# visinf/da-sac

Hardware: AMD Instinct MI355X
Metric: train images/sec (769x769, 19-cls, RN101 DeepLabv2, K=3) (higher is better)
Workload: dtype f32

## Files before the change

### da-sac_amd/csrc/winograd.hip

```cpp
#include "conv_common.hpp"
#include "winograd_index.hpp"

namespace dasac {
namespace wino {

constexpr int kBlock = 256;

__device__ __forceinline__ float ld(__amdgpu_buffer_rsrc_t r, unsigned voff) {
  return __uint_as_float(__builtin_amdgcn_raw_buffer_load_b32(r, voff, 0, 0));
}
__device__ __forceinline__ void st(__amdgpu_buffer_rsrc_t r, unsigned voff, float v) {
  __builtin_amdgcn_raw_buffer_store_b32(__float_as_uint(v), r, voff, 0, 0);
}

__global__ __launch_bounds__(kBlock) void filter_transform(const float* __restrict__ Wt, const float* __restrict__ scale,
                                                            float* __restrict__ U, int Cout, int Cin, int Mpad, int Kpad, int mode,
                                                            unsigned w_bytes, unsigned u_bytes) {
  const int idx = blockIdx.x * kBlock + threadIdx.x;
  const int per_point = Kpad * Mpad;
  if (idx >= per_point) return;
  const __amdgpu_buffer_rsrc_t rw = make_rsrc(Wt, w_bytes), ru = make_rsrc(U, u_bytes);
  const int row4 = Mpad * 4;
  const int kq = idx / row4, rem = idx - kq * row4;
  const int m = rem >> 2, k = kq * 4 + (rem & 3);
// ... 136 lines not shown
    for (int s = c; s < splits; s += 64) sv += ld(rs, (unsigned)(s * M + co) * 4u);
    sv = wave_sum(sv);
    if (c == 0) st(make_rsrc(sum_dz, (unsigned)M * 4u), (unsigned)co * 4u, sv);
  }
  __shared__ float red[4][16][64];
  __shared__ float grad[64 * 9];
  float acc[16];
#pragma unroll
  for (int pt = 0; pt < 16; ++pt) acc[pt] = 0.f;
  const unsigned point = (unsigned)(M * C), slab = 16u * point;
  const unsigned e0 = (unsigned)(co * C + ci0 + c);
  for (int s = q; s < splits; s += 4)
#pragma unroll
    for (int pt = 0; pt < 16; ++pt) acc[pt] += ld(rp, ((unsigned)s * slab + (unsigned)pt * point + e0) * 4u);
#pragma unroll
  for (int pt = 0; pt < 16; ++pt) red[q][pt][c] = acc[pt];
  __syncthreads();
  if (q == 0) {
    float p[4][4];
#pragma unroll
    for (int pt = 0; pt < 16; ++pt) p[pt >> 2][pt & 3] = (red[0][pt][c] + red[1][pt][c]) + (red[2][pt][c] + red[3][pt][c]);
    float r[3][4];
#pragma unroll
    for (int b = 0; b < 4; ++b) {
      r[0][b] = p[0][b] + 0.5f * (p[1][b] + p[2][b]);
      r[1][b] = 0.5f * (p[1][b] - p[2][b]);
      r[2][b] = 0.5f * (p[1][b] + p[2][b]) + p[3][b];
    }
#pragma unroll
    for (int a = 0; a < 3; ++a) {
      grad[c * 9 + a * 3 + 0] = r[a][0] + 0.5f * (r[a][1] + r[a][2]);
      grad[c * 9 + a * 3 + 1] = 0.5f * (r[a][1] - r[a][2]);
      grad[c * 9 + a * 3 + 2] = 0.5f * (r[a][1] + r[a][2]) + r[a][3];
    }
  }
  __syncthreads();
  const float sc = scale ? ld(make_rsrc(scale, (unsigned)M * 4u), (unsigned)co * 4u) : 1.f;
  float part = 0.f;
  for (int e = tx; e < 64 * 9; e += kBlock) {
    const unsigned off = ((unsigned)(co * C + ci0) * 9u + (unsigned)e) * 4u;
    if (dot) part += grad[e] * ld(rw, off);
    st(rd, off, grad[e] * sc);
  }
  if (dot) {
    __shared__ float redd[4];
    part = wave_sum(part);
    if (c == 0) redd[q] = part;
    __syncthreads();
    if (tx == 0) st(make_rsrc(dot, (unsigned)((C / 64) * M) * 4u), (unsigned)(blockIdx.x * M + co) * 4u, (redd[0] + redd[1]) + (redd[2] + redd[3]));
  }
}

}
}

using namespace dasac;
using dasac::wino::Geom;

static int wino_geom(Geom& g, const char* who, int Nb, int C, int M, int H, int W, int dilation) {
  DASAC_REQUIRE(Nb > 0 && C > 0 && M > 0 && H > 0 && W > 0 && dilation > 0, "%s: bad geometry", who);
  DASAC_REQUIRE((int64_t)Nb * H * W < (1ll << 30), "%s: more than 2^30 pixels", who);
  g = wino::make_geom(Nb, H, W, dilation);
  const int64_t cmax = C > M ? C : M;
  DASAC_REQUIRE(16 * cmax * (int64_t)g.T * 4 <= wino::kMaxBytes && cmax * (int64_t)Nb * H * W * 4 <= wino::kMaxBytes,
                "%s: a tensor exceeds the 4 GiB buffer-descriptor window", who);
  return DASAC_OK;
// ... 68 lines not shown

extern "C" int dasac_winograd_grad_input(const float* dz, int Nb, int M, int H, int W, int dilation, float* dm, size_t dm_bytes,
                                         dasac_stream_t stream) {
  DASAC_REQUIRE(dz && dm, "winograd_grad_input: null pointer");
  Geom g;
  const int rc = wino_geom(g, "winograd_grad_input", Nb, M, M, H, W, dilation);
  if (rc) return rc;
  DASAC_REQUIRE(M <= 65535, "winograd_grad_input: more than 65535 channels");
  const size_t need = (size_t)16 * M * g.T * 4;
  if (dm_bytes < need) return fail(DASAC_EWORKSPACE, "winograd_grad_input: workspace too small (%zu < %zu)", dm_bytes, need);
  hipLaunchKernelGGL(wino::grad_transform, dim3((g.T + wino::kBlock - 1) / wino::kBlock, M), dim3(wino::kBlock), 0, as_stream(stream), dz,
                     dm, g, M, (unsigned)((int64_t)Nb * M * H * W * 4), (unsigned)need);
  DASAC_CHECK_LAUNCH("winograd grad_transform");
  return DASAC_OK;
}

extern "C" int dasac_winograd_wgrad_finish(const void* workspace, size_t ws_bytes, int M, int C, int T, const float* w,
                                           const float* scale, float* dw, float* dot, float* sum_dz, dasac_stream_t stream) {
  DASAC_REQUIRE(workspace && w && dw, "winograd_wgrad_finish: null pointer");
  DASAC_REQUIRE(M > 0 && M <= 65535 && C > 0 && C % 64 == 0, "winograd_wgrad_finish: needs 1..65535 output channels and a multiple of 64 input channels");
  const int splits = dasac_conv_wgrad_batched_splits(16, M, C, T);
  DASAC_REQUIRE(splits > 0, "winograd_wgrad_finish: the batched weight-gradient launch does not take this shape");
  const size_t need = dasac_conv_wgrad_batched_workspace(16, M, C, T);
  if (ws_bytes < need) return fail(DASAC_EWORKSPACE, "winograd_wgrad_finish: workspace too small (%zu < %zu)", ws_bytes, need);
  const int64_t p_elems = (int64_t)splits * 16 * M * C;
  DASAC_REQUIRE(p_elems * 4 <= wino::kMaxBytes && (int64_t)M * C * 9 * 4 <= wino::kMaxBytes,
                "winograd_wgrad_finish: a tensor exceeds the 4 GiB buffer-descriptor window");
  const float* P = reinterpret_cast<const float*>(workspace);
  hipLaunchKernelGGL(wino::wgrad_finish, dim3(C / 64, M), dim3(wino::kBlock), 0, as_stream(stream), P, P + p_elems, splits, M, C, w, scale,
                     dw, dot, sum_dz, (unsigned)(p_elems * 4), (unsigned)((int64_t)M * C * 9 * 4));
  DASAC_CHECK_LAUNCH("winograd wgrad_finish");
  return DASAC_OK;
}
```

### da-sac_amd/csrc/winograd_index.hpp

```cpp
#pragma once
#include <stdint.h>

#if defined(__HIPCC__)
#define DASAC_HD __host__ __device__ __forceinline__
#else
#define DASAC_HD inline
#endif

namespace dasac {
namespace wino {

struct Div {
  unsigned mul, shift;
  int d;
};
DASAC_HD Div make_div(int d) {
  Div f{0u, 0u, d < 1 ? 1 : d};
  if (d <= 1) return f;
  int l = 1;
  while ((1ll << l) < d) ++l;
  const unsigned long long p = 1ull << (31 + l);
  f.mul = (unsigned)((p + (unsigned)d - 1) / (unsigned)d);
  f.shift = (unsigned)(l - 1);
  return f;
}
DASAC_HD int div(int n, Div f) {
  return f.mul ? (int)((unsigned)(((unsigned long long)(unsigned)n * f.mul) >> 32) >> f.shift) : n;
}

struct Axis {
  int n, d;
  int q, r;
  int b;
  int full;
  int tiles;
  Div by_d;
};
DASAC_HD Axis make_axis(int n, int d) {
  Axis a;
  a.n = n;
  a.d = d;
  a.q = n / d;
  a.r = n - a.q * d;
  a.b = (a.q + 1) / 2;
  a.full = a.b * d;
  a.tiles = a.full + ((a.q & 1) == 0 ? a.r : 0);
  a.by_d = make_div(d);
  return a;
}
DASAC_HD int phase_samples(const Axis& a, int p) { return a.q + (p < a.r ? 1 : 0); }
DASAC_HD void tile_decode(const Axis& a, int g, int& p, int& t) {
  if (g < a.full) {
    t = div(g, a.by_d);
    p = g - t * a.d;
  } else {
    t = a.b;
    p = g - a.full;
  }
}
DASAC_HD int tile_encode(const Axis& a, int p, int t) { return t < a.b ? t * a.d + p : a.full + p; }
DASAC_HD int first_out(const Axis& a, int p, int t) { return p + 2 * a.d * t; }
DASAC_HD void coord_to_tile(const Axis& a, int o, int& g, int& e) {
  const int i = div(o, a.by_d), p = o - i * a.d;
  e = i & 1;
  g = tile_encode(a, p, i >> 1);
}

struct Geom {
  Axis ay, ax;
  int N, H, W, HW;
  int tiles_img;
  int T;
  Div by_tiles_img, by_tx, by_hw, by_w;
};
DASAC_HD Geom make_geom(int N, int H, int W, int d) {
  Geom g;
  g.ay = make_axis(H, d);
  g.ax = make_axis(W, d);
  g.N = N;
  g.H = H;
  g.W = W;
  g.HW = H * W;
  g.tiles_img = g.ay.tiles * g.ax.tiles;
  g.T = N * g.tiles_img;
  g.by_tiles_img = make_div(g.tiles_img);
  g.by_tx = make_div(g.ax.tiles);
  g.by_hw = make_div(g.HW);
  g.by_w = make_div(W);
  return g;
}
DASAC_HD void tile_origin(const Geom& g, int tile, int& n, int& y0, int& x0) {
  n = div(tile, g.by_tiles_img);
  const int rem = tile - n * g.tiles_img;
  const int gy = div(rem, g.by_tx), gx = rem - gy * g.ax.tiles;
  int p, t;
  tile_decode(g.ay, gy, p, t);
  y0 = first_out(g.ay, p, t);
  tile_decode(g.ax, gx, p, t);
  x0 = first_out(g.ax, p, t);
}
DASAC_HD void pixel_tile(const Geom& g, int pix, int& n, int& rem, int& tile, int& ey, int& ex) {
  n = div(pix, g.by_hw);
  rem = pix - n * g.HW;
  const int y = div(rem, g.by_w), x = rem - y * g.W;
  int gy, gx;
  coord_to_tile(g.ay, y, gy, ey);
  coord_to_tile(g.ax, x, gx, ex);
  tile = (n * g.ay.tiles + gy) * g.ax.tiles + gx;
}

constexpr unsigned kOutside = 0xFFFFFFFFu;

DASAC_HD unsigned patch_offset(const Geom& g, int C, int n, int c, int y0, int x0, int ky, int kx) {
  const int y = y0 + (ky - 1) * g.ay.d, x = x0 + (kx - 1) * g.ax.d;
  if ((unsigned)y >= (unsigned)g.H || (unsigned)x >= (unsigned)g.W) return kOutside;
  return (unsigned)((n * C + c) * g.HW + y * g.W + x) * 4u;
}
DASAC_HD unsigned point_offset(const Geom& g, int C, int pt, int c, int tile) { return (unsigned)((pt * C + c) * g.T + tile) * 4u; }
DASAC_HD unsigned out_offset(const Geom& g, int M, int n, int m, int rem) { return (unsigned)((n * M + m) * g.HW + rem) * 4u; }
constexpr int64_t kMaxBytes = (1ll << 32) - 4096;

}
}
```

### da-sac_amd/dasac_hip/engine.py

```python
import torch

from . import ops
from . import lib as L


class ConvOp:
    kind = "conv"

    def __init__(self, src, dst, convs, bn, relu, res):
        c0 = convs[0]
        self.src, self.dst, self.res, self.relu = src, dst, res, bool(relu)
        self.convs, self.bn = list(convs), bn
        assert all(c.stride == c0.stride and c.in_channels == c0.in_channels and c.out_channels == c0.out_channels
                   and c.groups == 1 for c in convs)
        assert c0.stride[0] == c0.stride[1]
        branches = []
        for c in convs:
            assert c.dilation[0] == c.dilation[1] and c.padding[0] == c.padding[1]
            branches.append((c.kernel_size[0], c.kernel_size[1], c.dilation[0], c.padding[0]))
        self.spec = ops.ConvSpec(c0.in_channels, c0.out_channels, branches, c0.stride[0])
        self.has_bias = c0.bias is not None
        assert bn is None or len(convs) == 1
        self.expanded = ops.ExpandedConv(self.spec) if (len(convs) > 1 and c0.out_channels <= 32 and c0.stride[0] == 1) else None

# ... 96 lines not shown

    def _param_grads_expanded(self, eng, bp, d, dz, xin):
        need = bp.need
        if any(need[j] for j in self.w_idx):
            bp.store(self.w_idx, self.expanded.wgrad(d, xin, [c.weight.detach() for c in self.convs],
                                                     eng.table(self, xin.shape[2], xin.shape[3], False, xin.device),
                                                     outs=[bp.dest(j) for j in self.w_idx]))
        if any(need[j] for j in self.b_idx):
            bp.fan_out(self.b_idx, ops.channel_sums(dz, out=bp.sums_dest(self.b_idx, True, self.spec.cout, dz.device)))

    def _param_grads(self, eng, bp, i, dz, xin):
        spec, need, grads = self.spec, bp.need, bp.grads
        w_idx, b_idx, bn_idx = self.w_idx, self.b_idx, self.bn_idx
        train_bn = i in bp.aux
        want_bias = any(need[j] for j in b_idx)
        want_bn = any(need[j] for j in bn_idx)
        if train_bn:
            z, stats = bp.aux.pop(i)
            dz, dg, db = ops.bn_train_backward(dz, z, stats, self.bn.weight.detach(), want_params=want_bn,
                                               outs=(bp.dest(bn_idx[0]), bp.dest(bn_idx[1])) if want_bn else (None, None))
            del z
            if want_bn:
                bp.store(bn_idx, (dg, db))
            scale, invstd, want_bn = None, None, False
        else:
            scale, _, invstd = eng.fold(self)
        bias_is_sums = train_bn or self.bn is None
        sums, dot = None, None
        if any(need[j] for j in w_idx) or want_bn:
            if want_bn:
                dot = bp.dot_slice(spec, dz.device)
            if want_bn or want_bias:
                sums = bp.sums_dest(b_idx, want_bias and bias_is_sums, spec.cout, dz.device)
            if ops.winograd_wgrad_routed(spec, xin.shape[0], xin.shape[2], xin.shape[3]):
                bp.store(w_idx, [ops.winograd_wgrad(spec, dz, xin, self.convs[0].weight.detach(), scale=scale, dot=dot, sum_dz=sums,
                                                    out=bp.dest(w_idx[0]))])
            else:
                bp.store(w_idx, ops.conv_wgrad(spec, dz, xin, [c.weight.detach() for c in self.convs], scale=scale, dot=dot,
                                               table=eng.table(self, xin.shape[2], xin.shape[3], False, xin.device, wgrad=True),
                                               sum_dz=sums, outs=[bp.dest(j) for j in w_idx]))
        elif want_bias:
            sums = ops.channel_sums(dz, out=bp.sums_dest(b_idx, bias_is_sums, spec.cout, dz.device))
        if bias_is_sums:
            if want_bias:
                bp.fan_out(b_idx, sums)
        elif want_bn or want_bias:
            cb = self.convs[0].bias.detach() if self.has_bias else None
            dg, db, dcb = ops.bn_param_grads(dot, sums, self.bn.running_mean, invstd, scale, cb,
                                             want_gamma=want_bn, want_beta=want_bn, want_bias=want_bias,
                                             outs=(bp.dest(bn_idx[0]) if want_bn else None, bp.dest(bn_idx[1]) if want_bn else None,
                                                   bp.dest(b_idx[0]) if want_bias else None))
            if want_bn:
                bp.store(bn_idx, (dg, db))
            if want_bias:
                grads[b_idx[0]] = dcb
        return dz, scale


class PoolOp:
    kind = "pool"
    relu = False

    def __init__(self, src, dst, k, s, p, ceil_mode):
        self.src, self.dst, self.k, self.s, self.p, self.ceil = src, dst, k, s, p, bool(ceil_mode)

    def params(self):
        return []
# ... 625 lines not shown
```

### da-sac_amd/dasac_hip/lib.py

```python
import ctypes as C
import os

import torch

LIB_PATH = os.environ.get("DASAC_LIB") or os.path.join(os.path.dirname(os.path.abspath(__file__)), "libdasac_hip.so")

_p, _i, _l, _f, _sz = C.c_void_p, C.c_int, C.c_int64, C.c_float, C.c_size_t

PROTOTYPES = {
    "dasac_version": (_i, []),
    "dasac_last_error": (C.c_char_p, []),
    "dasac_device_info": (_i, [C.POINTER(_i), C.POINTER(_i), C.c_char_p, _sz]),
    "dasac_reserved_cus": (_i, []),
    "dasac_set_reserved_cus": (_i, [_i]),
    "dasac_pseudo_labels_workspace": (_sz, [_i, _i, _l]),
    "dasac_pseudo_labels": (_i, [_p, _p, _p, _f, _f, _i, _i, _l, _p, _p, _p, _p, _sz, _p]),
    "dasac_conv_mpad": (_i, [_i]),
    "dasac_conv_kpad": (_i, [_i]),
    "dasac_conv_table": (_i, [_p, _p, _p, _p, _i, _i, _i, _i, _i, _i, _p, _p]),
    "dasac_conv_pack": (_i, [_p, _p, _i, _i, _i, _i, _i, _i, _i, _p, _p]),
    "dasac_relu_bits_words": (_sz, [_i, _l]),
    "dasac_conv_gemm_bits_ok": (_i, [_i, _i]),
    "dasac_conv_gemm": (_i, [_p, _p, _p, _p] + [_i] * 12 + [_p, _p, _p, _p, _p, _i, _i, _i, _i, _p, _sz, _p]),
    "dasac_conv_gemm_batched": (_i, [_p, _p, _p, _p] + [_i] * 12 + [_i, _l, _l, _l, _p]),
# ... 36 lines not shown
    "dasac_adam_step_ctl": (_i, [_p, _i, _p, _i, _p, _i, C.c_double, C.c_double, C.c_double, _p, _i, _i, _p]),
    "dasac_tensor_stats_workspace": (_sz, [_i]),
    "dasac_tensor_stats": (_i, [_p, _i, _i, _p, _i, _p, _i, _p, _sz, _p, _p, _p, _p, _p, _p]),
    "dasac_activation_stats_workspace": (_sz, [_l]),
    "dasac_activation_stats": (_i, [_p, _i, _i, _i, _p, _i, _p, _sz, _p, _p]),
    "dasac_label_nodes": (_i, [_p, _i, _i, _i, _i, _i, _i, _i, _i, _p, _p]),
    "dasac_class_feature_stats_workspace": (_sz, [_i, _i, _i]),
    "dasac_class_feature_stats": (_i, [_p, _p, _i, _i, _i, _i, _p, _p, _p, _sz, _p]),
    "dasac_scale_planes": (_i, [_p, _p, _l, _l, _p, _p]),
    "dasac_add": (_i, [_p, _p, _p, _l, _p]),
    "dasac_relu_mask": (_i, [_p, _p, _p, _l, _p]),
    "dasac_bn_stats_workspace": (_sz, [_i, _i, _l]),
    "dasac_bn_stats": (_i, [_p, _i, _i, _l, _p, _p, _sz, _p]),
    "dasac_bn_train_finalize": (_i, [_p, C.c_double, _p, _p, _p, _p, _p, _p, _f, _f, _i, _p, _p, _p, _p, _p]),
    "dasac_bn_apply": (_i, [_p, _p, _p, _p, _i, _i, _i, _l, _p, _p]),
    "dasac_bn_bwd_reduce": (_i, [_p, _p, _p, _p, _i, _i, _l, _p, _p, _p, _p, _sz, _p]),
    "dasac_bn_train_finalize_tiles": (_i, [_p, _i, _i, C.c_double, _p, _p, _p, _p, _p, _f, _f, _i, _p, _p, _p, _p, _p]),
    "dasac_bn_tile_stats_reduce": (_i, [_p, _i, _i, _i, _p, _p]),
    "dasac_bn_train_apply_tiles": (_i, [_p, _p, _i, _i, C.c_double, _p, _p, _p, _p, _p, _f, _f, _p, _i, _i, _i, _l, _p, _p, _p, _p]),
    "dasac_bn_bwd_fused": (_i, [_p, _p, _p, _p, _p, C.c_double, _i, _i, _l, _p, _p, _p, _p, _sz, _p]),
    "dasac_conv_gemm_stats_ok": (_i, [_i, _i]),
    "dasac_conv_gemm_stats_tiles": (_i, [_i, _i, _i]),
    "dasac_conv_gemm_stats": (_i, [_p, _p, _p, _p] + [_i] * 12 + [_p, _p, _i, _i, _i, _i, _p, _sz, _p, _p]),
    "dasac_bn_bwd_apply": (_i, [_p, _p, _p, _p, _p, _p, C.c_double, _p, _i, _i, _l, _p, _p, _p, _p]),
    "dasac_winograd_tiles": (_i, [_i, _i, _i, _i]),
    "dasac_winograd_filter": (_i, [_p, _p, _i, _i, _i, _p, _p]),
    "dasac_winograd_input": (_i, [_p, _i, _i, _i, _i, _i, _p, _sz, _p]),
    "dasac_winograd_output": (_i, [_p, _sz, _i, _i, _i, _i, _i, _p, _i, _p, _p, _p, _p]),
    "dasac_winograd_grad_input": (_i, [_p, _i, _i, _i, _i, _i, _p, _sz, _p]),
    "dasac_conv_wgrad_batched_splits": (_i, [_i, _i, _i, _i]),
    "dasac_conv_wgrad_batched_workspace": (_sz, [_i, _i, _i, _i]),
    "dasac_conv_wgrad_batched": (_i, [_p, _p, _i, _i, _i, _i, _l, _l, _i, _p, _sz, _p]),
    "dasac_winograd_wgrad_finish": (_i, [_p, _sz, _i, _i, _i, _p, _p, _p, _p, _p, _p]),
    "dasac_conv_pack_expanded":(_i, [_p, _i, _i, _i, _i, _i, _i, _i, _p, _p]),
    "dasac_tap_gather": (_i, [_p, _p, _p, _p, _p, _i, _i, _i, _p, _i, _i, _i, _p, _p]),
    "dasac_tap_scatter": (_i, [_p, _p, _p, _p, _p, _i, _i, _i, _i, _i, _i, _p, _p]),
    "dasac_conv_wgrad_finish_expanded": (_i, [_p, _i, _i, _i, _i, _i, _p, _i, _i, _i, _i, _p]),
    "dasac_pack_chunk_elems": (_i, []),
    "dasac_bn_fold_multi": (_i, [_p, _p, _i, _p]),
    "dasac_conv_pack_multi": (_i, [_p, _p, _i, _p]),
    "dasac_label_pad_mask": (_i, [_p, _p, _l, _i, _i, _p]),
    "dasac_dropout_planes": (_i, [C.c_uint64, C.c_uint64, _f, _l, _p, _p]),
    "dasac_iou_counts": (_i, [_p, _p, _i, _i, _l, _i, _p, _p]),
    "dasac_mask_counts": (_i, [_p, _p, _p, _p, _p, _p, _p, _i, _i, _l, _i, _p, _p]),
    "dasac_confusion_counts": (_i, [_p, _p, _p, _p, _p, _p, _i, _p, _i, _i, _l, _i, _p, _p, _i, _i, _p]),
    "dasac_view_consistency": (_i, [_p, _i, _i, _i, _l, _f, _p, _p, _p, _p]),
    "dasac_boundary_counts_workspace": (_sz, [_i, _i, _i, _i]),
    "dasac_boundary_counts": (_i, [_p, _p, _p, _p, _p, _p, _i, _p, _i, _i, _i, _i, _i, _i, _p, _p, _sz, _p]),
    "dasac_label_hist": (_i, [_p, _i, _l, _p, _p]),
    "dasac_make_views_table_ints": (_i, [_i, _i]),
    "dasac_make_views": (_i, [_p, _p, _p, _i, _i, _i, _p, _p, _p, _i, _p, _p, _p, _p]),
    "dasac_view_photometric_workspace": (_sz, [_i, _i, _i]),
    "dasac_view_photometric": (_i, [_p, _p, _i, _i, _i, _p, _p, _p, _i, _p, _p, _p, _sz, _p]),
    "dasac_conv_wgrad_dot_rows": (_i, [_i, _i]),
    "dasac_conv_wgrad_finish": (_i, [_p, _i, _i, _i, _i, _i, _p, _p, _p, _p, _p, _i, _i, _i, _p]),
    "dasac_crop_table_ints": (_i, [_i, _i]),
    "dasac_resize_u8": (_i, [_p, _l, _p, _l, _i, _p, _p, _l, _i, _p, _l, _p, _l, _p]),
    "dasac_make_crops": (_i, [_p, _l, _p, _l, _i, _p, _p, _l, _i, _i, _p, _p, _i, _p, _p, _p, _p, _p, _p]),
    "dasac_vis_panels": (_i, [_p, _p, _i, _i, _i, _i, _i, _p, _p, _p, _p, _p, _p, _p]),
    "dasac_vis_grid": (_i, [_p, _i, _i, _i, _i, _f, _p, _p]),
}


class VisJob(C.Structure):
    _fields_ = [("src", _p), ("backdrop", _p), ("kind", C.c_int32), ("C", C.c_int32), ("H", C.c_int32), ("W", C.c_int32),
                ("softmax", C.c_int32), ("column", C.c_int32), ("column2", C.c_int32), ("reserved", C.c_int32)]
# ... 104 lines not shown
```

### da-sac_amd/dasac_hip/ops.py

```python
import os

import torch

from . import lib as L


def _c(t):
    return t if t.is_contiguous() else t.contiguous()


class _Profile:

    def __init__(self):
        self.on, self.records = False, []

    def start(self):
        self.on, self.records = True, []

    def stop(self, by_shape=False):
        self.on = False
        torch.cuda.synchronize()
        out = {}
        for name, flops, a, b, tag, nbytes in self.records:
            d = out.setdefault((name, tag) if by_shape else name, {"flops": 0.0, "bytes": 0.0, "seconds": 0.0, "launches": 0})
# ... 348 lines not shown
    lib = L.load()
    T = lib.dasac_winograd_tiles(Nb, H, W, spec.branches[0][2])
    return T > 0 and 64 * max(spec.cin, spec.cout) * T <= _MAX_TENSOR_BYTES \
        and lib.dasac_conv_wgrad_batched_splits(16, spec.cout, spec.cin, T) > 0


def winograd_wgrad(spec, dz, x, weight, scale=None, dot=None, sum_dz=None, out=None):
    lib = L.load()
    L.require_gpu(dz, x, weight, scale, dot, sum_dz)
    Nb, C, H, W = x.shape
    M, d = dz.shape[1], int(spec.branches[0][2])
    assert winograd_ok(spec) and (C, M) == (spec.cin, spec.cout) and tuple(dz.shape) == (Nb, M, H, W) and x.is_contiguous()
    assert dot is None or (tuple(dot.shape) == (dot_rows(spec), M) and dot.is_contiguous())
    T = lib.dasac_winograd_tiles(Nb, H, W, d)
    slab_bytes = lib.dasac_conv_wgrad_batched_workspace(16, M, C, T) if T > 0 else 0
    if slab_bytes == 0 or 64 * max(C, M) * T > _MAX_TENSOR_BYTES:
        raise L.DasacError("winograd_wgrad: {} x {} channels over {} tiles has no batched point contraction".format(M, C, T))
    v_elems, m_elems = 16 * C * T, 16 * M * T
    ws = L.workspace(4 * (v_elems + m_elems) + slab_bytes, x.device)
    v, dm, slabs = ws[:4 * v_elems], ws[4 * v_elems:4 * (v_elems + m_elems)], ws[4 * (v_elems + m_elems):]
    dz = _c(dz)
    with PROFILE.span("winograd_wgrad_input", 0.0, None, 4.0 * (x.numel() + v_elems)):
        L.check(lib.dasac_winograd_input(x.data_ptr(), Nb, C, H, W, d, v.data_ptr(), v.numel(), L.stream_ptr()), "dasac_winograd_input")
    with PROFILE.span("winograd_wgrad_grad", 0.0, None, 4.0 * (dz.numel() + m_elems)):
        L.check(lib.dasac_winograd_grad_input(dz.data_ptr(), Nb, M, H, W, d, dm.data_ptr(), dm.numel(), L.stream_ptr()),
                "dasac_winograd_grad_input")
    with PROFILE.span("winograd_wgrad_gemm", 2.0 * 16 * M * C * T, (M, C, T, 1, 1, False, False), 4.0 * (v_elems + m_elems + 16 * M * C)):
        L.check(lib.dasac_conv_wgrad_batched(dm.data_ptr(), v.data_ptr(), 16, M, C, T, M * T, C * T, 5, slabs.data_ptr(), slabs.numel(),
                                             L.stream_ptr()), "dasac_conv_wgrad_batched")
    dw = _dest(out, weight)
    with PROFILE.span("winograd_wgrad_finish", 0.0, None, float(slab_bytes) + 8.0 * weight.numel()):
        L.check(lib.dasac_winograd_wgrad_finish(slabs.data_ptr(), slabs.numel(), M, C, T, _c(weight).data_ptr(), L.ptr(scale), dw.data_ptr(),
                                                L.ptr(dot), L.ptr(sum_dz), L.stream_ptr()), "dasac_winograd_wgrad_finish")
    return dw


def dot_rows(spec):
    return L.load().dasac_conv_wgrad_dot_rows(spec.cin, spec.taps)


def conv_wgrad(spec, dz, x, weights, scale=None, dot=None, table=None, sum_dz=None, outs=None):
    lib = L.load()
    L.require_gpu(dz, x, *weights)
    assert dot is None or (tuple(dot.shape) == (dot_rows(spec), spec.cout) and dot.is_contiguous())
    Nb, Cx, H, W = x.shape
    _, M, OH, OW = dz.shape
    table = conv_table(spec, H, W, False, x.device) if table is None else table
    nbytes = lib.dasac_conv_wgrad_workspace(Nb, OH, OW, M, spec.K)
    ws = L.workspace(nbytes, x.device)
    with PROFILE.span("conv_wgrad", 2.0 * Nb * OH * OW * M * spec.K, (M, spec.K, Nb * OH * OW, spec.stride, 1, False, False),
                      4.0 * (dz.numel() + x.numel() + M * spec.K)):
        fn = lib.dasac_conv_wgrad_x3 if PRECISION == "bf16x3" else lib.dasac_conv_wgrad
        L.check(fn(_c(dz).data_ptr(), x.data_ptr(), table.data_ptr(), Nb, Cx, H, W, OH, OW, spec.stride, M,
                   spec.K, ws.data_ptr(), ws.numel(), L.stream_ptr()), "dasac_conv_wgrad")
    grads = [_dest(None if outs is None else outs[bi], w) for bi, w in enumerate(weights)]
    for w, dw, (taps, tap0) in zip(weights, grads, _branch_taps(spec)):
        L.check(lib.dasac_conv_wgrad_finish(ws.data_ptr(), Nb, OH, OW, M, spec.K, _c(w).data_ptr(), L.ptr(scale),
                                            dw.data_ptr(), L.ptr(dot), L.ptr(sum_dz if tap0 == 0 else None), spec.cin, taps,
                                            tap0, L.stream_ptr()),
                "dasac_conv_wgrad_finish")
    return grads


def _f32(shape, like):
    return torch.empty(shape, dtype=torch.float32, device=like.device)

# ... 1012 lines not shown
```

### include/dasac_hip.h

```cpp
#ifndef DASAC_HIP_H
#define DASAC_HIP_H

#include <stddef.h>
#include <stdint.h>

#ifdef __cplusplus
extern "C" {
#endif

#define DASAC_OK 0
#define DASAC_EINVAL (-1)
#define DASAC_EWORKSPACE (-2)
#define DASAC_ELAUNCH (-3)

typedef void* dasac_stream_t;

int dasac_version(void);
const char* dasac_last_error(void);
int dasac_device_info(int* cu_count, int* wave_size, char* arch, size_t arch_len);
int dasac_reserved_cus(void);
int dasac_set_reserved_cus(int n);

size_t dasac_pseudo_labels_workspace(int B, int C, int64_t HW);
int dasac_pseudo_labels(const float* probs, const uint8_t* ignore, const float* disc,
// ... 37 lines not shown
                          int OutH, int OutW, int ostride, const float* shift, const float* res, int relu,
                          int pix_begin, int pix_count, int schedule, void* workspace, size_t ws_bytes,
                          float* stats, dasac_stream_t stream);
size_t dasac_conv_gemm_workspace(void);
int dasac_conv_gemm_schedule(int Nb, int OH, int OW, int M, int K);
int dasac_conv_gemm_tail_split(int Nb, int OH, int OW, int M, int K);
size_t dasac_conv_wgrad_workspace(int Nb, int OH, int OW, int M, int K);
int dasac_conv_wgrad(const float* dz, const float* x, const int32_t* table,
                     int Nb, int Cx, int H, int W, int OH, int OW, int stride, int M, int K,
                     void* workspace, size_t ws_bytes, dasac_stream_t stream);
int dasac_conv_wgrad_x3(const float* dz, const float* x, const int32_t* table,
                        int Nb, int Cx, int H, int W, int OH, int OW, int stride, int M, int K,
                        void* workspace, size_t ws_bytes, dasac_stream_t stream);
int dasac_conv_wgrad_dot_rows(int Cin, int taps);
int dasac_conv_wgrad_finish(const void* workspace, int Nb, int OH, int OW, int M, int K,
                            const float* w, const float* scale, float* dw, float* dot,
                            float* sum_dz, int Cin, int taps, int tap0, dasac_stream_t stream);

int dasac_winograd_tiles(int Nb, int H, int W, int dilation);
int dasac_winograd_filter(const float* w, const float* scale, int Cout, int Cin, int transposed, float* u,
                          dasac_stream_t stream);
int dasac_winograd_input(const float* x, int Nb, int C, int H, int W, int dilation, float* v, size_t v_bytes,
                         dasac_stream_t stream);
int dasac_winograd_output(const float* y, size_t y_bytes, int Nb, int M, int H, int W, int dilation, const float* shift,
                          int relu, const uint32_t* mask_bits, uint32_t* relu_bits_out, float* out, dasac_stream_t stream);
int dasac_winograd_grad_input(const float* dz, int Nb, int M, int H, int W, int dilation, float* dm, size_t dm_bytes,
                              dasac_stream_t stream);
int dasac_conv_wgrad_batched_splits(int batch, int M, int C, int T);
size_t dasac_conv_wgrad_batched_workspace(int batch, int M, int C, int T);
int dasac_conv_wgrad_batched(const float* a, const float* b, int batch, int M, int C, int T, int64_t a_stride, int64_t b_stride,
                             int sum_entry, void* workspace, size_t ws_bytes, dasac_stream_t stream);
int dasac_winograd_wgrad_finish(const void* workspace, size_t ws_bytes, int M, int C, int T, const float* w, const float* scale,
                                float* dw, float* dot, float* sum_dz, dasac_stream_t stream);

int dasac_conv_pack_expanded(const float* w, int Cout, int Cin, int taps, int tap0, int total_taps,
                             int Cp, int transposed, float* packed, dasac_stream_t stream);
int dasac_tap_gather(const float* y, const int32_t* kh, const int32_t* kw, const int32_t* dil,
                     const int32_t* pad, int n_branches, int Cp, int Cout, const float* bias, int B,
                     int H, int W, float* out, dasac_stream_t stream);
int dasac_tap_scatter(const float* dout, const int32_t* kh, const int32_t* kw, const int32_t* dil,
                      const int32_t* pad, int n_branches, int Cp, int Cout, int B, int H, int W,
                      float* d, dasac_stream_t stream);
int dasac_conv_wgrad_finish_expanded(const void* workspace, int Nb, int OH, int OW, int E, int Cin,
                                     float* dw, int Cout, int taps, int tap0, int Cp,
                                     dasac_stream_t stream);

int dasac_upsample_softmax(const float* logits, int B, int C, int h, int w, int H, int W,
                           const uint8_t* ignore, float* up, float* probs, double* class_sums,
                           dasac_stream_t stream);
size_t dasac_upsample_bwd_workspace(int planes, int H, int w);
int dasac_upsample_bwd(const float* grad_up, int planes, int h, int w, int H, int W,
                       const float* gscale, float* grad_low, void* workspace, size_t ws_bytes,
                       dasac_stream_t stream);
size_t dasac_ce_loss_workspace(int B, int C, int64_t HW);
int dasac_ce_loss(const float* logits, const int64_t* labels, const float* class_weight,
                  const float* conf, int B, int C, int64_t HW, int mode, const float* gscale,
                  float* loss, float* dlogits, float* per_class, void* workspace, size_t ws_bytes,
                  dasac_stream_t stream);
size_t dasac_ce_loss_bwd_low_workspace(int B, int C, int H, int w);
int dasac_ce_loss_bwd_low(const float* logits_up, const int64_t* labels, const float* class_weight, const float* conf,
                          int B, int C, int H, int W, int h, int w, int mode, const float* gscale, float* grad_low,
                          void* workspace, size_t ws_bytes, dasac_stream_t stream);
int dasac_infer_labels(const float* logits, int B, int C, int h, int w, int H, int W, const uint8_t* lut,
                       uint8_t* labels, float* conf, dasac_stream_t stream);
#define DASAC_INFER_MAX_SOURCES 8
#define DASAC_INFER_MEAN 0
// ... 192 lines not shown
```

Measured before the change: 21.94.

## Add Winograd F(4x4,3x3) weight-gradient path for 256 and 512 channel convs

Adds a Winograd F(4,3) variant for the weight gradient of dilated 3x3 convolutions: 6x6 input and gradient transforms, a 36-point batched GEMM, and a finish kernel that applies the G^T transform. This covers roughly four times as many outputs per tile as the F(2,3) path, which cuts the number of tiles and the GEMM work per output. Routing applies only to 256x256 and 512x512 layers. In exchange it uses larger workspaces, adds precision risk from the fractional transform constants in fp32, and makes the finish kernel reduce 36 points.

```diff
diff --git a/da-sac_amd/csrc/winograd.hip b/da-sac_amd/csrc/winograd.hip
--- a/da-sac_amd/csrc/winograd.hip
+++ b/da-sac_amd/csrc/winograd.hip
@@ -192,6 +192,156 @@
       grad[c * 9 + a * 3 + 0] = r[a][0] + 0.5f * (r[a][1] + r[a][2]);
       grad[c * 9 + a * 3 + 1] = 0.5f * (r[a][1] - r[a][2]);
       grad[c * 9 + a * 3 + 2] = 0.5f * (r[a][1] + r[a][2]) + r[a][3];
+    }
+  }
+  __syncthreads();
+  const float sc = scale ? ld(make_rsrc(scale, (unsigned)M * 4u), (unsigned)co * 4u) : 1.f;
+  float part = 0.f;
+  for (int e = tx; e < 64 * 9; e += kBlock) {
+    const unsigned off = ((unsigned)(co * C + ci0) * 9u + (unsigned)e) * 4u;
+    if (dot) part += grad[e] * ld(rw, off);
+    st(rd, off, grad[e] * sc);
+  }
+  if (dot) {
+    __shared__ float redd[4];
+    part = wave_sum(part);
+    if (c == 0) redd[q] = part;
+    __syncthreads();
+    if (tx == 0) st(make_rsrc(dot, (unsigned)((C / 64) * M) * 4u), (unsigned)(blockIdx.x * M + co) * 4u, (redd[0] + redd[1]) + (redd[2] + redd[3]));
+  }
+}
+
+__device__ __forceinline__ void bt6(float d0, float d1, float d2, float d3, float d4, float d5, float (&o)[6]) {
+  o[0] = (2.f * (d0 + d4) + 3.f * (d1 - d3)) - 4.f * d2;
+  o[1] = (2.f * (d1 - d4) + 5.f * d2) + d3;
+  o[2] = (2.f * (d1 + d4) + d2) - 5.f * d3;
+  o[3] = (d3 - d1) + 2.f * (d4 - d2);
+  o[4] = 2.f * (d3 - d1) + (d2 - d4);
+  o[5] = (2.f * (d1 + d5) + 3.f * (d2 - d4)) - 4.f * d3;
+}
+__device__ __forceinline__ void a6(float y0, float y1, float y2, float y3, float (&o)[6]) {
+  o[0] = y0;
+  o[1] = (y0 + y2) + (y1 + y3);
+  o[2] = (y0 + y2) - (y1 + y3);
+  o[3] = (y0 + 4.f * y2) + (2.f * y1 + 8.f * y3);
+  o[4] = (y0 + 0.25f * y2) - (0.5f * y1 + 0.125f * y3);
+  o[5] = y3;
+}
+__device__ __forceinline__ void gt3(float p0, float p1, float p2, float p3, float p4, float p5, float (&o)[3]) {
+  constexpr float k6 = 1.f / 6.f, k15 = 1.f / 15.f, k30 = 1.f / 30.f;
+  o[0] = (0.5f * p0 + k6 * (p1 + p2)) + (k30 * p3 + (16.f * k15) * p4);
+  o[1] = k6 * (p1 - p2) + (k15 * p3 - (8.f * k15) * p4);
+  o[2] = (k6 * (p1 + p2) + 0.5f * p5) + ((2.f * k15) * p3 + (4.f * k15) * p4);
+}
+
+__global__ __launch_bounds__(kBlock) void input_transform4(const float* __restrict__ X, float* __restrict__ V, Geom g, int C,
+                                                            unsigned x_bytes, unsigned v_bytes) {
+  const int tile = blockIdx.x * kBlock + threadIdx.x;
+  if (tile >= g.T) return;
+  const int c = blockIdx.y;
+  const __amdgpu_buffer_rsrc_t rx = make_rsrc(X, x_bytes), rv = make_rsrc(V, v_bytes);
+  if (!real_tile(g, tile)) {
+#pragma unroll
+    for (int pt = 0; pt < 36; ++pt) st(rv, point_offset(g, C, pt, c, tile), 0.f);
+    return;
+  }
+  int n, y0, x0;
+  tile_origin<4>(g, tile, n, y0, x0);
+  float t[6][6];
+#pragma unroll
+  for (int kx = 0; kx < 6; ++kx) {
+    float d[6], o[6];
+#pragma unroll
+    for (int ky = 0; ky < 6; ++ky) d[ky] = ld(rx, patch_offset(g, C, n, c, y0, x0, ky, kx));
+    bt6(d[0], d[1], d[2], d[3], d[4], d[5], o);
+#pragma unroll
+    for (int a = 0; a < 6; ++a) t[a][kx] = o[a];
+  }
+#pragma unroll
+  for (int a = 0; a < 6; ++a) {
+    float v[6];
+    bt6(t[a][0], t[a][1], t[a][2], t[a][3], t[a][4], t[a][5], v);
+#pragma unroll
+    for (int b = 0; b < 6; ++b) st(rv, point_offset(g, C, a * 6 + b, c, tile), v[b]);
+  }
+}
+
+__global__ __launch_bounds__(kBlock) void grad_transform4(const float* __restrict__ dY, float* __restrict__ dM, Geom g, int M,
+                                                           unsigned y_bytes, unsigned m_bytes) {
+  const int tile = blockIdx.x * kBlock + threadIdx.x;
+  if (tile >= g.T) return;
+  const int m = blockIdx.y;
+  const __amdgpu_buffer_rsrc_t ry = make_rsrc(dY, y_bytes), rm = make_rsrc(dM, m_bytes);
+  if (!real_tile(g, tile)) {
+#pragma unroll
+    for (int pt = 0; pt < 36; ++pt) st(rm, point_offset(g, M, pt, m, tile), 0.f);
+    return;
+  }
+  int n, y0, x0;
+  tile_origin<4>(g, tile, n, y0, x0);
+  float t[6][4];
+#pragma unroll
+  for (int ex = 0; ex < 4; ++ex) {
+    float d[4], o[6];
+#pragma unroll
+    for (int ey = 0; ey < 4; ++ey) d[ey] = ld(ry, patch_offset(g, M, n, m, y0, x0, ey + 1, ex + 1));
+    a6(d[0], d[1], d[2], d[3], o);
+#pragma unroll
+    for (int a = 0; a < 6; ++a) t[a][ex] = o[a];
+  }
+#pragma unroll
+  for (int a = 0; a < 6; ++a) {
+    float v[6];
+    a6(t[a][0], t[a][1], t[a][2], t[a][3], v);
+#pragma unroll
+    for (int b = 0; b < 6; ++b) st(rm, point_offset(g, M, a * 6 + b, m, tile), v[b]);
+  }
+}
+
+__global__ __launch_bounds__(kBlock) void wgrad_finish4(const float* __restrict__ P, const float* __restrict__ Psum, int splits, int M,
+                                                         int C, const float* __restrict__ Wt, const float* __restrict__ scale,
+                                                         float* __restrict__ dW, float* __restrict__ dot, float* __restrict__ sum_dz,
+                                                         unsigned p_bytes, unsigned w_bytes) {
+  const int co = blockIdx.y, ci0 = blockIdx.x * 64;
+  const int tx = threadIdx.x, c = tx & 63, q = tx >> 6;
+  const __amdgpu_buffer_rsrc_t rp = make_rsrc(P, p_bytes), rw = make_rsrc(Wt, w_bytes), rd = make_rsrc(dW, w_bytes);
+  if (sum_dz && blockIdx.x == 0 && q == 0) {
+    const __amdgpu_buffer_rsrc_t rs = make_rsrc(Psum, (unsigned)(splits * M) * 4u);
+    float sv = 0.f;
+    for (int s = c; s < splits; s += 64) sv += ld(rs, (unsigned)(s * M + co) * 4u);
+    sv = wave_sum(sv);
+    if (c == 0) st(make_rsrc(sum_dz, (unsigned)M * 4u), (unsigned)co * 4u, sv);
+  }
+  __shared__ float red[4][36][64];
+  __shared__ float grad[64 * 9];
+  float acc[36];
+#pragma unroll
+  for (int pt = 0; pt < 36; ++pt) acc[pt] = 0.f;
+  const unsigned point = (unsigned)(M * C), slab = 36u * point;
+  const unsigned e0 = (unsigned)(co * C + ci0 + c);
+  for (int s = q; s < splits; s += 4)
+#pragma unroll
+    for (int pt = 0; pt < 36; ++pt) acc[pt] += ld(rp, ((unsigned)s * slab + (unsigned)pt * point + e0) * 4u);
+#pragma unroll
+  for (int pt = 0; pt < 36; ++pt) red[q][pt][c] = acc[pt];
+  __syncthreads();
+  if (q == 0) {
+    float r[3][6];
+#pragma unroll
+    for (int b = 0; b < 6; ++b) {
+      float p[6], o[3];
+#pragma unroll
+      for (int a = 0; a < 6; ++a) p[a] = (red[0][a * 6 + b][c] + red[1][a * 6 + b][c]) + (red[2][a * 6 + b][c] + red[3][a * 6 + b][c]);
+      gt3(p[0], p[1], p[2], p[3], p[4], p[5], o);
+#pragma unroll
+      for (int a = 0; a < 3; ++a) r[a][b] = o[a];
+    }
+#pragma unroll
+    for (int a = 0; a < 3; ++a) {
+      float o[3];
+      gt3(r[a][0], r[a][1], r[a][2], r[a][3], r[a][4], r[a][5], o);
+#pragma unroll
+      for (int b = 0; b < 3; ++b) grad[c * 9 + a * 3 + b] = o[b];
     }
   }
   __syncthreads();
@@ -326,3 +476,64 @@
   DASAC_CHECK_LAUNCH("winograd wgrad_finish");
   return DASAC_OK;
 }
+
+static int wino_geom4(Geom& g, const char* who, int Nb, int C, int H, int W, int dilation) {
+  DASAC_REQUIRE(Nb > 0 && C > 0 && C <= 65535 && H > 0 && W > 0 && dilation > 0, "%s: bad geometry", who);
+  DASAC_REQUIRE((int64_t)Nb * H * W < (1ll << 30), "%s: more than 2^30 pixels", who);
+  g = wino::make_geom<4>(Nb, H, W, dilation);
+  DASAC_REQUIRE(36 * (int64_t)C * g.T * 4 <= wino::kMaxBytes && (int64_t)C * Nb * H * W * 4 <= wino::kMaxBytes,
+                "%s: a tensor exceeds the 4 GiB buffer-descriptor window", who);
+  return DASAC_OK;
+}
+
+extern "C" int dasac_winograd4_tiles(int Nb, int H, int W, int dilation) {
+  if (Nb <= 0 || H <= 0 || W <= 0 || dilation <= 0) return 0;
+  const int64_t t = (int64_t)Nb * wino::make_axis<4>(H, dilation).tiles * wino::make_axis<4>(W, dilation).tiles;
+  return t < (1ll << 30) ? (int)((t + 3) / 4 * 4) : 0;
+}
+
+extern "C" int dasac_winograd4_input(const float* x, int Nb, int C, int H, int W, int dilation, float* v, size_t v_bytes,
+                                     dasac_stream_t stream) {
+  DASAC_REQUIRE(x && v, "winograd4_input: null pointer");
+  Geom g;
+  const int rc = wino_geom4(g, "winograd4_input", Nb, C, H, W, dilation);
+  if (rc) return rc;
+  const size_t need = (size_t)36 * C * g.T * 4;
+  if (v_bytes < need) return fail(DASAC_EWORKSPACE, "winograd4_input: workspace too small (%zu < %zu)", v_bytes, need);
+  hipLaunchKernelGGL(wino::input_transform4, dim3((g.T + wino::kBlock - 1) / wino::kBlock, C), dim3(wino::kBlock), 0, as_stream(stream), x,
+                     v, g, C, (unsigned)((int64_t)Nb * C * H * W * 4), (unsigned)need);
+  DASAC_CHECK_LAUNCH("winograd input_transform4");
+  return DASAC_OK;
+}
+
+extern "C" int dasac_winograd4_grad_input(const float* dz, int Nb, int M, int H, int W, int dilation, float* dm, size_t dm_bytes,
+                                          dasac_stream_t stream) {
+  DASAC_REQUIRE(dz && dm, "winograd4_grad_input: null pointer");
+  Geom g;
+  const int rc = wino_geom4(g, "winograd4_grad_input", Nb, M, H, W, dilation);
+  if (rc) return rc;
+  const size_t need = (size_t)36 * M * g.T * 4;
+  if (dm_bytes < need) return fail(DASAC_EWORKSPACE, "winograd4_grad_input: workspace too small (%zu < %zu)", dm_bytes, need);
+  hipLaunchKernelGGL(wino::grad_transform4, dim3((g.T + wino::kBlock - 1) / wino::kBlock, M), dim3(wino::kBlock), 0, as_stream(stream), dz,
+                     dm, g, M, (unsigned)((int64_t)Nb * M * H * W * 4), (unsigned)need);
+  DASAC_CHECK_LAUNCH("winograd grad_transform4");
+  return DASAC_OK;
+}
+
+extern "C" int dasac_winograd4_wgrad_finish(const void* workspace, size_t ws_bytes, int M, int C, int T, const float* w,
+                                            const float* scale, float* dw, float* dot, float* sum_dz, dasac_stream_t stream) {
+  DASAC_REQUIRE(workspace && w && dw, "winograd4_wgrad_finish: null pointer");
+  DASAC_REQUIRE(M > 0 && M <= 65535 && C > 0 && C % 64 == 0, "winograd4_wgrad_finish: needs 1..65535 output channels and a multiple of 64 input channels");
+  const int splits = dasac_conv_wgrad_batched_splits(36, M, C, T);
+  DASAC_REQUIRE(splits > 0, "winograd4_wgrad_finish: the batched weight-gradient launch does not take this shape");
+  const size_t need = dasac_conv_wgrad_batched_workspace(36, M, C, T);
+  if (ws_bytes < need) return fail(DASAC_EWORKSPACE, "winograd4_wgrad_finish: workspace too small (%zu < %zu)", ws_bytes, need);
+  const int64_t p_elems = (int64_t)splits * 36 * M * C;
+  DASAC_REQUIRE(p_elems * 4 <= wino::kMaxBytes && (int64_t)M * C * 9 * 4 <= wino::kMaxBytes,
+                "winograd4_wgrad_finish: a tensor exceeds the 4 GiB buffer-descriptor window");
+  const float* P = reinterpret_cast<const float*>(workspace);
+  hipLaunchKernelGGL(wino::wgrad_finish4, dim3(C / 64, M), dim3(wino::kBlock), 0, as_stream(stream), P, P + p_elems, splits, M, C, w, scale,
+                     dw, dot, sum_dz, (unsigned)(p_elems * 4), (unsigned)((int64_t)M * C * 9 * 4));
+  DASAC_CHECK_LAUNCH("winograd wgrad_finish4");
+  return DASAC_OK;
+}
diff --git a/da-sac_amd/csrc/winograd_index.hpp b/da-sac_amd/csrc/winograd_index.hpp
--- a/da-sac_amd/csrc/winograd_index.hpp
+++ b/da-sac_amd/csrc/winograd_index.hpp
@@ -36,15 +36,17 @@
   int tiles;
   Div by_d;
 };
+template <int TM = 2>
 DASAC_HD Axis make_axis(int n, int d) {
+  static_assert(TM == 2 || TM == 4, "outputs per tile and axis: 2 or 4 (coord_to_tile shifts by log2)");
   Axis a;
   a.n = n;
   a.d = d;
   a.q = n / d;
   a.r = n - a.q * d;
-  a.b = (a.q + 1) / 2;
+  a.b = (a.q + TM - 1) / TM;
   a.full = a.b * d;
-  a.tiles = a.full + ((a.q & 1) == 0 ? a.r : 0);
+  a.tiles = a.full + ((a.q & (TM - 1)) == 0 ? a.r : 0);
   a.by_d = make_div(d);
   return a;
 }
@@ -59,11 +61,13 @@
   }
 }
 DASAC_HD int tile_encode(const Axis& a, int p, int t) { return t < a.b ? t * a.d + p : a.full + p; }
-DASAC_HD int first_out(const Axis& a, int p, int t) { return p + 2 * a.d * t; }
+template <int TM = 2>
+DASAC_HD int first_out(const Axis& a, int p, int t) { return p + TM * a.d * t; }
+template <int TM = 2>
 DASAC_HD void coord_to_tile(const Axis& a, int o, int& g, int& e) {
   const int i = div(o, a.by_d), p = o - i * a.d;
-  e = i & 1;
-  g = tile_encode(a, p, i >> 1);
+  e = i & (TM - 1);
+  g = tile_encode(a, p, i >> (TM == 4 ? 2 : 1));
 }
 
 struct Geom {
@@ -73,39 +77,43 @@
   int T;
   Div by_tiles_img, by_tx, by_hw, by_w;
 };
+template <int TM = 2>
 DASAC_HD Geom make_geom(int N, int H, int W, int d) {
   Geom g;
-  g.ay = make_axis(H, d);
-  g.ax = make_axis(W, d);
+  g.ay = make_axis<TM>(H, d);
+  g.ax = make_axis<TM>(W, d);
   g.N = N;
   g.H = H;
   g.W = W;
   g.HW = H * W;
   g.tiles_img = g.ay.tiles * g.ax.tiles;
-  g.T = N * g.tiles_img;
+  g.T = TM == 4 ? (N * g.tiles_img + 3) / 4 * 4 : N * g.tiles_img;
   g.by_tiles_img = make_div(g.tiles_img);
   g.by_tx = make_div(g.ax.tiles);
   g.by_hw = make_div(g.HW);
   g.by_w = make_div(W);
   return g;
 }
+template <int TM = 2>
 DASAC_HD void tile_origin(const Geom& g, int tile, int& n, int& y0, int& x0) {
   n = div(tile, g.by_tiles_img);
   const int rem = tile - n * g.tiles_img;
   const int gy = div(rem, g.by_tx), gx = rem - gy * g.ax.tiles;
   int p, t;
   tile_decode(g.ay, gy, p, t);
-  y0 = first_out(g.ay, p, t);
+  y0 = first_out<TM>(g.ay, p, t);
   tile_decode(g.ax, gx, p, t);
-  x0 = first_out(g.ax, p, t);
+  x0 = first_out<TM>(g.ax, p, t);
 }
+DASAC_HD bool real_tile(const Geom& g, int tile) { return tile < g.N * g.tiles_img; }
+template <int TM = 2>
 DASAC_HD void pixel_tile(const Geom& g, int pix, int& n, int& rem, int& tile, int& ey, int& ex) {
   n = div(pix, g.by_hw);
   rem = pix - n * g.HW;
   const int y = div(rem, g.by_w), x = rem - y * g.W;
   int gy, gx;
-  coord_to_tile(g.ay, y, gy, ey);
-  coord_to_tile(g.ax, x, gx, ex);
+  coord_to_tile<TM>(g.ay, y, gy, ey);
+  coord_to_tile<TM>(g.ax, x, gx, ex);
   tile = (n * g.ay.tiles + gy) * g.ax.tiles + gx;
 }
 
diff --git a/da-sac_amd/dasac_hip/engine.py b/da-sac_amd/dasac_hip/engine.py
--- a/da-sac_amd/dasac_hip/engine.py
+++ b/da-sac_amd/dasac_hip/engine.py
@@ -152,7 +152,10 @@
                 dot = bp.dot_slice(spec, dz.device)
             if want_bn or want_bias:
                 sums = bp.sums_dest(b_idx, want_bias and bias_is_sums, spec.cout, dz.device)
-            if ops.winograd_wgrad_routed(spec, xin.shape[0], xin.shape[2], xin.shape[3]):
+            if ops.winograd4_wgrad_routed(spec, xin.shape[0], xin.shape[2], xin.shape[3]):
+                bp.store(w_idx, [ops.winograd4_wgrad(spec, dz, xin, self.convs[0].weight.detach(), scale=scale, dot=dot, sum_dz=sums,
+                                                     out=bp.dest(w_idx[0]))])
+            elif ops.winograd_wgrad_routed(spec, xin.shape[0], xin.shape[2], xin.shape[3]):
                 bp.store(w_idx, [ops.winograd_wgrad(spec, dz, xin, self.convs[0].weight.detach(), scale=scale, dot=dot, sum_dz=sums,
                                                     out=bp.dest(w_idx[0]))])
             else:
diff --git a/da-sac_amd/dasac_hip/lib.py b/da-sac_amd/dasac_hip/lib.py
--- a/da-sac_amd/dasac_hip/lib.py
+++ b/da-sac_amd/dasac_hip/lib.py
@@ -92,6 +92,10 @@
     "dasac_conv_wgrad_batched_workspace": (_sz, [_i, _i, _i, _i]),
     "dasac_conv_wgrad_batched": (_i, [_p, _p, _i, _i, _i, _i, _l, _l, _i, _p, _sz, _p]),
     "dasac_winograd_wgrad_finish": (_i, [_p, _sz, _i, _i, _i, _p, _p, _p, _p, _p, _p]),
+    "dasac_winograd4_tiles": (_i, [_i, _i, _i, _i]),
+    "dasac_winograd4_input": (_i, [_p, _i, _i, _i, _i, _i, _p, _sz, _p]),
+    "dasac_winograd4_grad_input": (_i, [_p, _i, _i, _i, _i, _i, _p, _sz, _p]),
+    "dasac_winograd4_wgrad_finish": (_i, [_p, _sz, _i, _i, _i, _p, _p, _p, _p, _p, _p]),
     "dasac_conv_pack_expanded":(_i, [_p, _i, _i, _i, _i, _i, _i, _i, _p, _p]),
     "dasac_tap_gather": (_i, [_p, _p, _p, _p, _p, _i, _i, _i, _p, _i, _i, _i, _p, _p]),
     "dasac_tap_scatter": (_i, [_p, _p, _p, _p, _p, _i, _i, _i, _i, _i, _i, _p, _p]),
diff --git a/da-sac_amd/dasac_hip/ops.py b/da-sac_amd/dasac_hip/ops.py
--- a/da-sac_amd/dasac_hip/ops.py
+++ b/da-sac_amd/dasac_hip/ops.py
@@ -404,6 +404,54 @@
     with PROFILE.span("winograd_wgrad_finish", 0.0, None, float(slab_bytes) + 8.0 * weight.numel()):
         L.check(lib.dasac_winograd_wgrad_finish(slabs.data_ptr(), slabs.numel(), M, C, T, _c(weight).data_ptr(), L.ptr(scale), dw.data_ptr(),
                                                 L.ptr(dot), L.ptr(sum_dz), L.stream_ptr()), "dasac_winograd_wgrad_finish")
+    return dw
+
+
+WINOGRAD4_WGRAD_LAYERS = {(256, 256), (512, 512)}
+WINOGRAD4_MIN_SAMPLES = 8
+
+
+def winograd4_wgrad_routed(spec, Nb, H, W):
+    if ALGORITHM != "auto" or not winograd_ok(spec) or spec.cin * spec.cout < WINOGRAD_WGRAD_MIN_CHANNEL_PRODUCT:
+        return False
+    if spec.cin % 128 or spec.cout % 128 or (spec.cin, spec.cout) not in WINOGRAD4_WGRAD_LAYERS:
+        return False
+    d = spec.branches[0][2]
+    if H // d < WINOGRAD4_MIN_SAMPLES or W // d < WINOGRAD4_MIN_SAMPLES:
+        return False
+    lib = L.load()
+    T = lib.dasac_winograd4_tiles(Nb, H, W, d)
+    return T > 0 and 144 * max(spec.cin, spec.cout) * T <= _MAX_TENSOR_BYTES \
+        and lib.dasac_conv_wgrad_batched_splits(36, spec.cout, spec.cin, T) > 0
+
+
+def winograd4_wgrad(spec, dz, x, weight, scale=None, dot=None, sum_dz=None, out=None):
+    lib = L.load()
+    L.require_gpu(dz, x, weight, scale, dot, sum_dz)
+    Nb, C, H, W = x.shape
+    M, d = dz.shape[1], int(spec.branches[0][2])
+    assert winograd_ok(spec) and (C, M) == (spec.cin, spec.cout) and tuple(dz.shape) == (Nb, M, H, W) and x.is_contiguous()
+    assert dot is None or (tuple(dot.shape) == (dot_rows(spec), M) and dot.is_contiguous())
+    T = lib.dasac_winograd4_tiles(Nb, H, W, d)
+    slab_bytes = lib.dasac_conv_wgrad_batched_workspace(36, M, C, T) if T > 0 else 0
+    if slab_bytes == 0 or 144 * max(C, M) * T > _MAX_TENSOR_BYTES:
+        raise L.DasacError("winograd4_wgrad: {} x {} channels over {} tiles has no batched point contraction".format(M, C, T))
+    v_elems, m_elems = 36 * C * T, 36 * M * T
+    ws = L.workspace(4 * (v_elems + m_elems) + slab_bytes, x.device)
+    v, dm, slabs = ws[:4 * v_elems], ws[4 * v_elems:4 * (v_elems + m_elems)], ws[4 * (v_elems + m_elems):]
+    dz = _c(dz)
+    with PROFILE.span("winograd4_wgrad_input", 0.0, None, 4.0 * (x.numel() + v_elems)):
+        L.check(lib.dasac_winograd4_input(x.data_ptr(), Nb, C, H, W, d, v.data_ptr(), v.numel(), L.stream_ptr()), "dasac_winograd4_input")
+    with PROFILE.span("winograd4_wgrad_grad", 0.0, None, 4.0 * (dz.numel() + m_elems)):
+        L.check(lib.dasac_winograd4_grad_input(dz.data_ptr(), Nb, M, H, W, d, dm.data_ptr(), dm.numel(), L.stream_ptr()),
+                "dasac_winograd4_grad_input")
+    with PROFILE.span("winograd4_wgrad_gemm", 2.0 * 36 * M * C * T, (M, C, T, 1, 1, False, False), 4.0 * (v_elems + m_elems + 36 * M * C)):
+        L.check(lib.dasac_conv_wgrad_batched(dm.data_ptr(), v.data_ptr(), 36, M, C, T, M * T, C * T, 7, slabs.data_ptr(), slabs.numel(),
+                                             L.stream_ptr()), "dasac_conv_wgrad_batched")
+    dw = _dest(out, weight)
+    with PROFILE.span("winograd4_wgrad_finish", 0.0, None, float(slab_bytes) + 8.0 * weight.numel()):
+        L.check(lib.dasac_winograd4_wgrad_finish(slabs.data_ptr(), slabs.numel(), M, C, T, _c(weight).data_ptr(), L.ptr(scale), dw.data_ptr(),
+                                                 L.ptr(dot), L.ptr(sum_dz), L.stream_ptr()), "dasac_winograd4_wgrad_finish")
     return dw
 
 
diff --git a/include/dasac_hip.h b/include/dasac_hip.h
--- a/include/dasac_hip.h
+++ b/include/dasac_hip.h
@@ -93,6 +93,13 @@
                              int sum_entry, void* workspace, size_t ws_bytes, dasac_stream_t stream);
 int dasac_winograd_wgrad_finish(const void* workspace, size_t ws_bytes, int M, int C, int T, const float* w, const float* scale,
                                 float* dw, float* dot, float* sum_dz, dasac_stream_t stream);
+int dasac_winograd4_tiles(int Nb, int H, int W, int dilation);
+int dasac_winograd4_input(const float* x, int Nb, int C, int H, int W, int dilation, float* v, size_t v_bytes,
+                          dasac_stream_t stream);
+int dasac_winograd4_grad_input(const float* dz, int Nb, int M, int H, int W, int dilation, float* dm, size_t dm_bytes,
+                               dasac_stream_t stream);
+int dasac_winograd4_wgrad_finish(const void* workspace, size_t ws_bytes, int M, int C, int T, const float* w, const float* scale,
+                                 float* dw, float* dot, float* sum_dz, dasac_stream_t stream);
 
 int dasac_conv_pack_expanded(const float* w, int Cout, int Cin, int taps, int tap0, int total_taps,
                              int Cp, int transposed, float* packed, dasac_stream_t stream);
```

Result: faster. 22.46 (median of 6 runs) (+2.4%).
